# slyforce/MusicStyleTransfer

Measured on AMD Instinct MI355X. Metric: piano-roll frames/s (VAE train step), higher is better.
Workload: dtype bf16; 1 GPU; BASELINE configs[1]: single-track piano-roll VAE train step, T=256, pitch=128, latent=64, batch=64/GPU, bf16; encoder 256x2x8h, decoder 128x1x8h (scripts/train-vae.sh), dropout 0.2; Xavier-initialised weights; global_batch=64, seq_len=256, pitches=128, latent=64, parallelism=dp1, params=1885440

## Files before the change

include/mst_hip.h:

```cpp
#ifndef MST_HIP_H
#define MST_HIP_H

#include <stdint.h>

#ifdef __cplusplus
extern "C" {
#endif

typedef void* mst_stream_t;

enum mst_status {
  MST_OK = 0,
  MST_ERR_INVALID = -1,
  MST_ERR_LAUNCH = -2,
  MST_ERR_UNSUPPORTED = -3
};

enum mst_dtype { MST_BF16 = 0, MST_F16 = 1, MST_F32 = 2 };

enum mst_act { MST_ACT_NONE = 0, MST_ACT_RELU = 1 };

int mst_version(void);
const char* mst_last_error(void);
int mst_device_count(void);
// ... 135 lines not shown
                     int64_t S_out, int64_t s_off, const int32_t* idx, float* dst, int64_t ldd,
                     float alpha, mst_stream_t stream);

int mst_mask_from_lengths(int64_t B, int64_t S, const int32_t* lens, int32_t add,
                          uint8_t* keymask, mst_stream_t stream);

int mst_attn_keysoftmax_fwd(int dtype, int64_t B, int64_t S, int64_t H, int64_t dh,
                            const void* qkv, int64_t ld_qkv, int64_t k_off, int64_t q_off, int64_t v_off,
                            const uint8_t* keymask, float* lse,
                            void* out, int64_t ld_out,
                            int64_t q_limit ,
                            mst_stream_t stream);

int mst_attn_qkv_fwd(int dtype, int64_t B, int64_t S, int64_t H, int64_t dh, const void* x, int64_t ld_x, const void* w,
                     int64_t ld_w, const float* bias, void* qkv, int64_t ld_qkv, int64_t k_off, int64_t q_off, int64_t v_off,
                     const uint8_t* keymask, float* lse, void* out, int64_t ld_out, int64_t q_limit, mst_stream_t stream);
int mst_attn_keysoftmax_bwd(int dtype, int64_t B, int64_t S, int64_t H, int64_t dh,
                            const void* qkv, int64_t ld_qkv, int64_t k_off, int64_t q_off, int64_t v_off,
                            const uint8_t* keymask, const float* lse,
                            const void* dout, int64_t ld_dout,
                            void* dqkv, int64_t ld_dqkv, float* delta,
                            int64_t q_limit ,
                            mst_stream_t stream);

int mst_attn_causal_fwd(int dtype, int64_t B, int64_t S, int64_t H, int64_t dh,
                        const void* qkv, int64_t ld_qkv, int64_t k_off, int64_t q_off, int64_t v_off,
                        const uint8_t* keymask, float* lse, void* out, int64_t ld_out, mst_stream_t stream);
int mst_attn_causal_bwd(int dtype, int64_t B, int64_t S, int64_t H, int64_t dh,
                        const void* qkv, int64_t ld_qkv, int64_t k_off, int64_t q_off, int64_t v_off,
                        const uint8_t* keymask, const float* lse, const void* dout, int64_t ld_dout,
                        void* dqkv, int64_t ld_dqkv, float* delta, mst_stream_t stream);

int mst_layernorm_fwd(int dtype, int64_t M, int64_t D, const void* x, int64_t ldx,
                      const float* gamma, const float* beta, float eps,
                      void* y, int64_t ldy, float* mean, float* rstd,
                      int64_t row_id_stride ,
                      mst_stream_t stream);

int mst_layernorm_bwd(int dtype, int64_t M, int64_t D, const void* x, int64_t ldx,
                      const float* gamma, const float* mean, const float* rstd,
                      const void* dy, int64_t ldy, void* dx, int64_t ld_dx,
                      void* dx_masked, int64_t ld_dxm, float* dgamma, float* dbeta,
                      int mask_mode, float dropout_p, uint64_t dropout_seed, uint32_t dropout_site,
                      const uint64_t* dropout_seed_ptr,
                      int64_t row_id_stride ,
                      float* partials ,
// ... 191 lines not shown
```

musicstyletransfer_amd/_lib.py:

```python
import ctypes as C
import os

HERE = os.path.dirname(os.path.abspath(__file__))
LIB_PATH = os.path.join(HERE, "csrc", "libmst_hip.so")

MST_BF16, MST_F16, MST_F32 = 0, 1, 2
ACT_NONE, ACT_RELU = 0, 1
CE_MAX_WORKGROUPS = 4096

c_i32, c_i64, c_f32, c_f64, c_u64, c_u32 = C.c_int32, C.c_int64, C.c_float, C.c_double, C.c_uint64, C.c_uint32
vp = C.c_void_p


class GemmArgs(C.Structure):
    _fields_ = [
        ("dtype", c_i32), ("c_f32", c_i32),
        ("M", c_i64), ("N", c_i64), ("K", c_i64),
        ("A", vp), ("lda", c_i64),
        ("B", vp), ("ldb", c_i64),
        ("C", vp), ("ldc", c_i64),
        ("bias", vp),
        ("resid", vp), ("ldr", c_i64),
        ("act", c_i32),
        ("gate", vp), ("ldg", c_i64),
# ... 152 lines not shown
    "mst_gemm_wgrad": (C.c_int, [C.POINTER(WgradArgs), vp]),
    "mst_gemm_wgrad_batch": (C.c_int, [C.POINTER(WgradArgs), C.c_int, vp]),
    "mst_gemm_wgrad_batch_ws": (C.c_int, [C.POINTER(WgradArgs), C.c_int, vp, c_i64, vp]),
    "mst_gemm_wgrad_batch_sums": (C.c_int, [C.POINTER(WgradArgs), C.c_int, vp, c_i64, C.POINTER(PartialSum), C.c_int, vp]),
    "mst_gemm_wgrad_batch_flush": (C.c_int, [C.POINTER(WgradArgs), C.c_int, vp, c_i64, C.POINTER(PartialSum), C.c_int,
                                             C.POINTER(OuterJob), C.c_int, vp]),
    "mst_outer_jobs": (C.c_int, [C.POINTER(OuterJob), C.c_int, vp]),
    "mst_latent_bwd_vec": (C.c_int, [C.c_int, c_i64, c_i64, c_i64, c_i64, vp, vp, vp, vp, vp, vp, vp, c_i64, c_f32, c_f32, c_f32,
                                     c_f32, vp, c_i64, vp, c_i64, vp, vp]),
    "mst_latent_bwd_vec_proj": (C.c_int, [C.c_int, c_i64, c_i64, c_i64, c_i64, vp, vp, vp, vp, vp, vp, vp, c_i64, vp, c_i64, c_i64, vp, c_i64,
                                          c_f32, c_f32, c_f32, c_f32, vp, c_i64, vp, c_i64, vp, vp]),
    "mst_embed_fwd": (C.c_int, [C.c_int, c_i64, c_i64, c_i64, vp, vp, c_i64, vp, vp, c_i64, vp, c_i64, c_f32,
                                vp, c_i64, c_i64, c_i64, vp, vp]),
    "mst_embed_bwd": (C.c_int, [C.c_int, c_i64, c_i64, c_i64, vp, vp, c_i64, vp, vp, c_i64, c_f32,
                                vp, c_i64, c_i64, c_i64, vp]),
    "mst_group_colsum": (C.c_int, [C.c_int, c_i64, c_i64, c_i64, vp, c_i64, c_i64, c_i64, vp, vp, c_i64, c_f32, vp]),
    "mst_mask_from_lengths": (C.c_int, [c_i64, c_i64, vp, c_i32, vp, vp]),
    "mst_attn_keysoftmax_fwd": (C.c_int, [C.c_int, c_i64, c_i64, c_i64, c_i64, vp, c_i64, c_i64, c_i64, c_i64,
                                          vp, vp, vp, c_i64, c_i64, vp]),
    "mst_attn_qkv_fwd": (C.c_int, [C.c_int, c_i64, c_i64, c_i64, c_i64, vp, c_i64, vp, c_i64, vp, vp, c_i64, c_i64, c_i64, c_i64, vp, vp, vp,
                                   c_i64, c_i64, vp]),
    "mst_attn_keysoftmax_bwd": (C.c_int, [C.c_int, c_i64, c_i64, c_i64, c_i64, vp, c_i64, c_i64, c_i64, c_i64,
                                          vp, vp, vp, c_i64, vp, c_i64, vp, c_i64, vp]),
    "mst_attn_causal_fwd": (C.c_int, [C.c_int, c_i64, c_i64, c_i64, c_i64, vp, c_i64, c_i64, c_i64, c_i64, vp, vp, vp, c_i64, vp]),
    "mst_attn_causal_bwd": (C.c_int, [C.c_int, c_i64, c_i64, c_i64, c_i64, vp, c_i64, c_i64, c_i64, c_i64,
                                      vp, vp, vp, c_i64, vp, c_i64, vp, vp]),
    "mst_attn_decode": (C.c_int, [C.c_int, c_i64, c_i64, c_i64, c_i64, c_i64, vp, c_i64, c_i64, c_i64, c_i64, C.c_int, vp, c_i64, vp]),
    "mst_layernorm_fwd": (C.c_int, [C.c_int, c_i64, c_i64, vp, c_i64, vp, vp, c_f32, vp, c_i64, vp, vp, c_i64, vp]),
    "mst_layernorm_bwd": (C.c_int, [C.c_int, c_i64, c_i64, vp, c_i64, vp, vp, vp, vp, c_i64, vp, c_i64,
                                    vp, c_i64, vp, vp, C.c_int, c_f32, c_u64, c_u32, vp, c_i64, vp, vp]),
    "mst_latent_fwd": (C.c_int, [C.c_int, c_i64, c_i64, c_i64, c_i64, vp, c_i64, vp, vp, vp, vp, vp, vp, vp, c_i64,
                                 vp, c_f32, vp, vp, vp, vp, vp, c_i64, vp]),
    "mst_latent_fwd_proj": (C.c_int, [C.c_int, c_i64, c_i64, c_i64, c_i64, vp, c_i64, vp, vp, vp, vp, vp, vp, vp, c_i64,
                                      vp, c_f32, vp, vp, vp, vp, vp, c_i64, vp, c_i64, vp, vp, c_i64, c_i64, vp]),
    "mst_latent_bwd": (C.c_int, [C.c_int, c_i64, c_i64, c_i64, c_i64, vp, c_i64, vp, vp, vp, vp, vp, vp, vp,
                                 vp, c_i64, c_f32, c_f32, c_f32, c_f32, vp, vp, vp, vp, vp, c_i64, vp, c_i64, vp, vp]),
    "mst_reparam_kl_fwd": (C.c_int, [c_i64, c_i64, vp, vp, vp, vp, vp, vp]),
    "mst_reparam_kl_bwd": (C.c_int, [c_i64, c_i64, vp, vp, vp, vp, c_f32, vp, vp, vp]),
    "mst_softmax_ce": (C.c_int, [C.c_int, c_i64, c_i64, c_i64, vp, c_i64, vp, vp, vp, c_i64, vp, c_i64, c_f32, C.c_int, vp,
                                 C.c_int, vp]),
    "mst_ce_from_probs": (C.c_int, [C.c_int, c_i64, c_i64, c_i64, vp, c_i64, vp, vp, vp]),
    "mst_bce_from_probs": (C.c_int, [C.c_int, c_i64, c_i64, vp, vp, c_f32, C.c_int, vp, vp]),
    "mst_sigmoid_bce": (C.c_int, [C.c_int, c_i64, c_i64, c_i64, vp, c_i64, vp, c_f32, C.c_int, vp, vp, vp, c_i64,
                                  vp, c_i64, c_f32, C.c_int, vp]),
    "mst_beam_step": (C.c_int, [c_i64, c_i64, c_i64, c_i64, c_i64, vp, c_i64, vp, vp, vp, vp, vp, vp, vp, c_i32, c_i32, vp]),
    "mst_beam_gather": (C.c_int, [vp, vp, vp, c_i64, c_i64, c_i64, c_i64, vp]),
# ... 61 lines not shown
```

musicstyletransfer_amd/csrc/attention.hip:

```cpp
#include <math.h>
#include <stdlib.h>
#include <type_traits>
#include "common.hpp"

namespace mst {

#ifndef MST_ATT_STAGE
#define MST_ATT_STAGE 64
#endif
template <int DH> struct Stage { static constexpr int ROWS = MST_ATT_STAGE; };
template <int DH> struct LdsLd { static constexpr int V = DH + 8; };
constexpr int ATT_WG_ROWS = 128;
constexpr float MASK_VALUE = -1e9f;
constexpr float NEG_BIG = -3.0e38f;
constexpr float LOG2E = 1.4426950408889634f;

__device__ __forceinline__ void key_consts(bool in_range, bool valid_key, float rmax, float logl, float scale, float& sk2,
                                           float& ck2) {
  if (!in_range) { sk2 = 0.f; ck2 = -INFINITY; }
  else if (!valid_key) { sk2 = 0.f; ck2 = -logl * LOG2E; }
  else { sk2 = scale * LOG2E; ck2 = -(rmax + logl) * LOG2E; }
}
__device__ __forceinline__ float fast_exp2(float x) { return __builtin_amdgcn_exp2f(x); }
#define MST_FOR_TILES(kt, bits) for (uint64_t mst_m_ = (bits); mst_m_; mst_m_ &= mst_m_ - 1) if (const int kt = __builtin_ctzll(mst_m_); true)
// ... 832 lines not shown
    __syncthreads();
    LOOP_STAMP(6 + 5 * kc);
  }
  ATT_STAMP(1);
  if (!active) return;
  const bool in = row < S;
  T* const tiles[3] = {sK, sQ, sV};
  T* qrow = reinterpret_cast<T*>(const_cast<void*>(a.qkv)) + (b * S + row) * a.ld_qkv + hd * DH;
#pragma unroll
  for (int c = 0; c < 3; ++c) {
#pragma unroll
    for (int g = 0; g < 4; ++g) {
      u32x2 o = {0u, 0u};
      if (in) {
        o[0] = (uint32_t)f32_to_bits<T>(acc[c][4 * g]) | ((uint32_t)f32_to_bits<T>(acc[c][4 * g + 1]) << 16);
        o[1] = (uint32_t)f32_to_bits<T>(acc[c][4 * g + 2]) | ((uint32_t)f32_to_bits<T>(acc[c][4 * g + 3]) << 16);
        *reinterpret_cast<u32x2*>(qrow + sec_off[c] + 8 * g + h4) = o;
      }
      *reinterpret_cast<u32x2*>(tiles[c] + row * LD + 8 * g + h4) = o;
    }
  }
}

template <typename T, int DH, bool QKV = false, bool CHUNKED = false>
__global__ __launch_bounds__((FWD_MAX_WAVES<DH, QKV || CHUNKED> * 64)) __attribute__((amdgpu_waves_per_eu((DH == 16 ? MST_ATT16_WAVES_FWD : (FWD_MAX_WAVES<DH, QKV || CHUNKED> == 8 ? 2 : 4))))) void attn_fwd_res_kernel(AttnArgs a) {
  constexpr int KS = DH / 16, DB = (DH + 31) / 32, LD = LdsLd<DH>::V;
  extern __shared__ __attribute__((aligned(16))) unsigned char att_smem[];
  const int64_t S = a.S;
  const int NB = (int)((S + 31) / 32), SP = NB * 32;
  const bool restage = !QKV && a.restage;
  const int CR = CHUNKED ? SP / a.restage : SP;
  T* sQ = reinterpret_cast<T*>(att_smem);
  T* sK = restage ? sQ : sQ + SP * LD;
  T* sV = sK + CR * LD;
  float* sSk = reinterpret_cast<float*>(CHUNKED ? sQ + SP * LD : sV + SP * LD);
  float* sCk = sSk + SP; float* sMadd = sCk + SP; float* sMax = sMadd + SP; float* sLogl = sMax + SP;
  float* sRed = sLogl + SP;
  const int tid = threadIdx.x, lane = tid & 63, wave = tid >> 6, nthr = blockDim.x, NW = nthr >> 6;
  const int64_t bh = res_wg_bh(a.B, a.H), b = (int64_t)((uint32_t)bh / (uint32_t)a.H), hd = bh - b * a.H;
  const int64_t plane = a.B * a.H * S;
  const bool lone = lone_row_shape(S, DH) && a.q_limit >= S;
  const int NBo = lone ? NB - 1 : NB;
  const T* base = reinterpret_cast<const T*>(a.qkv) + b * S * a.ld_qkv + hd * DH;
  ATT_STAMP(0);
  if constexpr (QKV) {
    static_assert(DH == 32, "the fused projection is built for head size 32");
// ... 158 lines not shown
      for (int f = 0; f < DH; ++f) acc[f] = 0.f;
      for (int k = tid; k < S; k += nthr) {
        const float x = lds_row_dot<T, DH>(sK + k * LD, qe);
        const float p = exact ? exact_prob(x, a.scale, sMadd[k], sMax[k], sLogl[k]) : fast_exp2(fmaf(x, sSk[k], sCk[k]));
        lds_row_axpy<T, DH>(p, sV + k * LD, acc);
      }
#pragma unroll
      for (int f = 0; f < DH; ++f) acc[f] = wave_sum(acc[f]);
      if (lane == 0) {
#pragma unroll
        for (int f = 0; f < DH; ++f) sRed[wave * DH + f] = acc[f];
      }
      __syncthreads();
      if (tid < DH) {
        float o_e = 0.f;
        for (int w = 0; w < NW; ++w) o_e += sRed[w * DH + tid];
        T* og = reinterpret_cast<T*>(a.out) + b * S * a.ld_out + hd * DH;
        og[e * a.ld_out + tid] = (T)o_e;
      }
    }
  }
}

template <typename T, int DH, bool SPARSE>
__global__ __launch_bounds__(RES_MAX_WAVES<DH> * 64) __attribute__((amdgpu_waves_per_eu(DH == 16 ? MST_ATT16_WAVES_BWD : (DH == 64 ? 2 : 4)))) void attn_bwd_res_kernel(AttnArgs a) {
  constexpr int KS = DH / 16, DB = (DH + 31) / 32, LD = LdsLd<DH>::V;
  extern __shared__ __attribute__((aligned(16))) unsigned char att_smem[];
  const int64_t S = a.S;
  const int NB = (int)((S + 31) / 32), SP = NB * 32;
  T* bufA = reinterpret_cast<T*>(att_smem);
  T* bufB = bufA + SP * LD;
  float* sSk = reinterpret_cast<float*>(bufB + SP * LD);
  float* sCk = sSk + SP; float* sMadd = sCk + SP; float* sMax = sMadd + SP; float* sLogl = sMax + SP; float* sNd = sLogl + SP;
  float* sRed = sNd + SP;
  const int tid = threadIdx.x, lane = tid & 63, wave = tid >> 6, nthr = blockDim.x, NW = nthr >> 6;
  const int64_t bh = res_wg_bh(a.B, a.H), b = (int64_t)((uint32_t)bh / (uint32_t)a.H), hd = bh - b * a.H;
  const int64_t plane = a.B * a.H * S;
  const bool lone = !SPARSE && lone_row_shape(S, DH);
  const int NBo = lone ? NB - 1 : NB;
  const float log2_scale = __log2f(a.scale);
  const T* base = reinterpret_cast<const T*>(a.qkv) + b * S * a.ld_qkv + hd * DH;
  const T* Kg = base + a.k_off;
  const T* Qg = base + a.q_off;
  const T* Vg = base + a.v_off;
  const T* dOg = reinterpret_cast<const T*>(a.dout) + b * S * a.ld_dout + hd * DH;
  T* dbase = reinterpret_cast<T*>(a.dqkv) + b * S * a.ld_dqkv + hd * DH;
  constexpr bool sparse = SPARSE;
  const int64_t do_rows = sparse ? a.q_limit : S;
  typename Act<T>::vec8 kf[KS], vf[KS];
#pragma unroll
  for (int s = 0; s < KS; ++s) {
    kf[s] = glb_row_frag<T>(Kg, a.ld_qkv, wave * 32 + (lane & 31), S, s, lane);
    vf[s] = glb_row_frag<T>(Vg, a.ld_qkv, wave * 32 + (lane & 31), S, s, lane);
  }
  ATT_STAMP(0);
  stage_pair<T, DH>(bufA, Qg, a.ld_qkv, S, bufB, dOg, a.ld_dout, do_rows, SP, tid, nthr);
  __syncthreads();
  ATT_STAMP(1);
  const int nq0 = sparse ? 1 : NBo;

  int padded = 0;
  for (int ob = wave; ob < NBo; ob += NW) {
    const int64_t k_lane = ob * 32 + (lane & 31);
    if (ob != wave) {
#pragma unroll
      for (int s = 0; s < KS; ++s) {
        kf[s] = glb_row_frag<T>(Kg, a.ld_qkv, k_lane, S, s, lane);
        vf[s] = glb_row_frag<T>(Vg, a.ld_qkv, k_lane, S, s, lane);
      }
    }
    const bool in = k_lane < S;
    const bool vk = in && a.keymask[b * S + k_lane];
    const float rmax = in ? a.lse[bh * S + k_lane] : 0.f;
    const float logl = in ? a.lse[plane + bh * S + k_lane] : INFINITY;
    const float madd = vk ? 0.f : MASK_VALUE;
    float sk2, ck2;
    key_consts(in, vk, rmax, in ? logl : 0.f, a.scale, sk2, ck2);
    const float ck2s = ck2 + log2_scale;
    const bool exact_w = __any(in && !vk);
// ... 91 lines not shown
      }
      __syncthreads();
      if (tid < DH) {
        float dk = 0.f;
        for (int w = 0; w < NW; ++w) dk += sRed[w * DH + tid];
        dbase[e * a.ld_dqkv + a.k_off + tid] = (T)dk;
      }
      if (tid == 0) {
        a.delta[bh * S + e] = delta;
        sSk[e] = sk2; sCk[e] = ck2s; sMadd[e] = madd; sMax[e] = rmax; sLogl[e] = logl; sNd[e] = -delta;
        for (int k = (int)S; k < SP; ++k) {
          float s0, c0;
          key_consts(false, false, 0.f, 0.f, a.scale, s0, c0);
          sSk[k] = s0; sCk[k] = c0 + log2_scale; sMadd[k] = MASK_VALUE; sMax[k] = 0.f; sLogl[k] = INFINITY; sNd[k] = 0.f;
        }
      }
    }
  }
  ATT_STAMP(3);
  typename Act<T>::vec8 qf[KS], dof[KS];
#pragma unroll
  for (int s = 0; s < KS; ++s) {
    qf[s] = glb_row_frag<T>(Qg, a.ld_qkv, wave * 32 + (lane & 31), S, s, lane);
    dof[s] = glb_row_frag<T>(dOg, a.ld_dout, wave * 32 + (lane & 31), do_rows, s, lane);
  }
  __syncthreads();
  stage_pair<T, DH>(bufA, Kg, a.ld_qkv, S, bufB, Vg, a.ld_qkv, S, SP, tid, nthr);
  const bool exact = __syncthreads_or(padded);
  const uint64_t pad_tiles = exact ? padded_tile_mask(sSk, sCk, NB, lane) : 0ull;
  ATT_STAMP(4);

  for (int ob = wave; ob < NBo; ob += NW) {
    const int64_t q_lane = ob * 32 + (lane & 31);
    if (ob != wave) {
#pragma unroll
      for (int s = 0; s < KS; ++s) {
        qf[s] = glb_row_frag<T>(Qg, a.ld_qkv, q_lane, S, s, lane);
        dof[s] = glb_row_frag<T>(dOg, a.ld_dout, q_lane, do_rows, s, lane);
      }
    }
    f32x16 acc[DB];
#pragma unroll
    for (int d = 0; d < DB; ++d) acc[d] = zero16<DH>();
    if (sparse && ob > 0) {
      if (exact) {
        MST_FOR_TILES(kt, ~pad_tiles & tile_bits(NB)) bwd_q_tile<T, DH, false, true>(bufA, bufB, sSk, sCk, sMadd, sMax, sLogl, sNd, kt, a.scale, qf, dof, acc, lane);
        MST_FOR_TILES(kt, pad_tiles & tile_bits(NB)) bwd_q_tile<T, DH, true, true>(bufA, bufB, sSk, sCk, sMadd, sMax, sLogl, sNd, kt, a.scale, qf, dof, acc, lane);
      } else for (int kt = 0; kt < NB; ++kt) bwd_q_tile<T, DH, false, true>(bufA, bufB, sSk, sCk, sMadd, sMax, sLogl, sNd, kt, a.scale, qf, dof, acc, lane);
    } else if (exact) {
      MST_FOR_TILES(kt, ~pad_tiles & tile_bits(NBo)) bwd_q_tile<T, DH, false>(bufA, bufB, sSk, sCk, sMadd, sMax, sLogl, sNd, kt, a.scale, qf, dof, acc, lane);
      MST_FOR_TILES(kt, pad_tiles & tile_bits(NBo)) bwd_q_tile<T, DH, true>(bufA, bufB, sSk, sCk, sMadd, sMax, sLogl, sNd, kt, a.scale, qf, dof, acc, lane);
    } else {
      for (int kt = 0; kt < NBo; ++kt) bwd_q_tile<T, DH, false>(bufA, bufB, sSk, sCk, sMadd, sMax, sLogl, sNd, kt, a.scale, qf, dof, acc, lane);
    }
    if constexpr (DH <= 16 && !SPARSE) {
      if (lone) {
        if (exact) bwd_q_tile<T, DH, true, false, true>(bufA, bufB, sSk, sCk, sMadd, sMax, sLogl, sNd, NB - 1, a.scale, qf, dof, acc, lane);
        else bwd_q_tile<T, DH, false, false, true>(bufA, bufB, sSk, sCk, sMadd, sMax, sLogl, sNd, NB - 1, a.scale, qf, dof, acc, lane);
      }
    }
    owner_store<T, DH>(q_lane < S ? dbase + a.q_off + q_lane * a.ld_dqkv : nullptr, acc, lane);
  }
  ATT_STAMP(5);
  if constexpr (DH <= 16 && !SPARSE) {
    if (lone) {
      const int64_t e = S - 1;
      float qe[DH], doe[DH], acc[DH];
#pragma unroll
      for (int f = 0; f < DH; ++f) { qe[f] = to_f32(Qg[e * a.ld_qkv + f]); doe[f] = to_f32(dOg[e * a.ld_dout + f]); acc[f] = 0.f; }
      for (int k = tid; k < S; k += nthr) {
        const float x = lds_row_dot<T, DH>(bufA + k * LD, qe);
        const float ps = exact ? exact_prob(x, a.scale, sMadd[k], sMax[k], sLogl[k]) * a.scale : fast_exp2(fmaf(x, sSk[k], sCk[k]));
        const float dl = ps * (lds_row_dot<T, DH>(bufB + k * LD, doe) + sNd[k]);
        lds_row_axpy<T, DH>(dl, bufA + k * LD, acc);
      }
#pragma unroll
      for (int f = 0; f < DH; ++f) acc[f] = wave_sum(acc[f]);
      if (lane == 0) {
#pragma unroll
        for (int f = 0; f < DH; ++f) sRed[wave * DH + f] = acc[f];
      }
      __syncthreads();
      if (tid < DH) {
        float dq = 0.f;
        for (int w = 0; w < NW; ++w) dq += sRed[w * DH + tid];
        dbase[e * a.ld_dqkv + a.q_off + tid] = (T)dq;
      }
    }
  }
}

template <typename T, int DH, int OBM>
// ... 212 lines not shown
    const int NB = (int)cdiv(a.S, 32);
    if (!off && DH == 32 && NB <= OBM * NWQ) {
      for (int nc = 1; nc <= 4; nc *= 2) {
        if (NB % nc != 0) break;
        const size_t lds = (size_t)2 * (NB * 32 / nc) * LdsLd<DH>::V * 2 + (size_t)6 * NB * 32 * 4;
        if (lds > 150 * 1024) continue;
        static size_t attr_lds = 64 * 1024;
        if (lds > attr_lds) {
          const hipError_t e = hipFuncSetAttribute(reinterpret_cast<const void*>(&attn_bwd_q_chunk_kernel<T, DH, OBM>), hipFuncAttributeMaxDynamicSharedMemorySize, (int)lds);
          if (e != hipSuccess) { set_error("attn_bwd_q_chunk_kernel: LDS opt-in of %zu bytes: %s", lds, hipGetErrorString(e)); return MST_ERR_LAUNCH; }
          attr_lds = lds;
        }
        hipLaunchKernelGGL((attn_bwd_q_chunk_kernel<T, DH, OBM>), dim3((unsigned)(a.B * a.H)), dim3(NWQ * 64), lds, s, a, nc);
        MST_CHECK_LAUNCH("attn_bwd_q_chunk_kernel");
        return MST_OK;
      }
    }
  }
  hipLaunchKernelGGL((attn_bwd_q_kernel<T, DH>), grid, dim3(256), 0, s, a);
  MST_CHECK_LAUNCH("attn_bwd_q_kernel");
  return MST_OK;
}


template <typename T, int DH>
__global__ __launch_bounds__(64) void attn_decode_kernel(int64_t H, int64_t n_keys, int64_t t_max, const T* __restrict__ cache,
                                                          int64_t ld, int64_t k_off, int64_t q_off, int64_t v_off, int mode,
                                                          float scale, T* __restrict__ out, int64_t ld_out) {
  const int64_t b = blockIdx.x / H, hd = blockIdx.x % H;
  const int lane = threadIdx.x;
  const T* base = cache + b * t_max * ld + hd * DH;
  float q[DH];
#pragma unroll
  for (int d = 0; d < DH; ++d) q[d] = to_f32(base[(n_keys - 1) * ld + q_off + d]);
  float m = -INFINITY;
  if (mode == 1) {
    for (int64_t k = lane; k < n_keys; k += 64) {
      float l = 0.f;
#pragma unroll
      for (int d = 0; d < DH; ++d) l = fmaf(to_f32(base[k * ld + k_off + d]), q[d], l);
      m = fmaxf(m, l * scale);
    }
    m = wave_max(m);
  }
  float acc[DH], z = 0.f;
#pragma unroll
// ... 88 lines not shown
extern "C" int mst_attn_keysoftmax_bwd(int dtype, int64_t B, int64_t S, int64_t H, int64_t dh, const void* qkv,
                                       int64_t ld_qkv, int64_t k_off, int64_t q_off, int64_t v_off,
                                       const uint8_t* keymask, const float* lse, const void* dout, int64_t ld_dout,
                                       void* dqkv, int64_t ld_dqkv, float* delta, int64_t q_limit, mst_stream_t stream) {
  int rc = attn_check(B, S, H, dh, ld_qkv, k_off, q_off, v_off);
  if (rc) return rc;
  MST_CHECK_ARG(qkv && keymask && lse && dout && dqkv && delta, "mst_attn_keysoftmax_bwd: null pointer");
  MST_CHECK_ARG(ld_dout % 8 == 0 && ld_dout >= H * dh && ld_dqkv % 8 == 0, "mst_attn_keysoftmax_bwd: bad leading dims");
  AttnArgs a = {};
  a.B = B; a.S = S; a.H = H; a.qkv = qkv; a.ld_qkv = ld_qkv; a.k_off = k_off; a.q_off = q_off; a.v_off = v_off;
  a.keymask = keymask; a.lse = const_cast<float*>(lse); a.dout = dout; a.ld_dout = ld_dout; a.dqkv = dqkv;
  a.ld_dqkv = ld_dqkv; a.delta = delta;
  a.q_limit = (q_limit > 0 && q_limit < S) ? q_limit : 0;
  a.scale = 1.f / sqrtf((float)dh);
  hipStream_t s = (hipStream_t)stream;
  return dispatch_act(dtype, [&](auto tag) -> int {
    typedef decltype(tag) T;
    if (dh == 16) return launch_bwd<T, 16>(a, s);
    if (dh == 32) return launch_bwd<T, 32>(a, s);
    return launch_bwd<T, 64>(a, s);
  });
}

extern "C" int mst_attn_decode(int dtype, int64_t B, int64_t H, int64_t dh, int64_t n_keys, int64_t t_max, const void* cache,
                               int64_t ld, int64_t k_off, int64_t q_off, int64_t v_off, int mode, void* out, int64_t ld_out,
                               mst_stream_t stream) {
  MST_CHECK_ARG(B > 0 && H > 0 && n_keys > 0 && n_keys <= t_max && cache && out, "mst_attn_decode: bad argument");
  MST_CHECK_ARG(dh == 16 || dh == 32 || dh == 64, "mst_attn_decode: head size must be 16, 32 or 64 (got %lld)", (long long)dh);
  MST_CHECK_ARG(mode == 0 || mode == 1, "mst_attn_decode: mode must be 0 (softmax over the query axis, the reference) or 1 (over the keys)");
  MST_CHECK_ARG(ld_out >= H * dh, "mst_attn_decode: ld_out < H*dh");
  const float scale = 1.f / sqrtf((float)dh);
  hipStream_t s = (hipStream_t)stream;
  return dispatch_act(dtype, [&](auto tag) -> int {
    typedef decltype(tag) T;
    const dim3 grid((unsigned)(B * H));
    if (dh == 16) hipLaunchKernelGGL((attn_decode_kernel<T, 16>), grid, dim3(64), 0, s, H, n_keys, t_max, (const T*)cache, ld, k_off, q_off, v_off, mode, scale, (T*)out, ld_out);
    else if (dh == 32) hipLaunchKernelGGL((attn_decode_kernel<T, 32>), grid, dim3(64), 0, s, H, n_keys, t_max, (const T*)cache, ld, k_off, q_off, v_off, mode, scale, (T*)out, ld_out);
    else hipLaunchKernelGGL((attn_decode_kernel<T, 64>), grid, dim3(64), 0, s, H, n_keys, t_max, (const T*)cache, ld, k_off, q_off, v_off, mode, scale, (T*)out, ld_out);
    MST_CHECK_LAUNCH("attn_decode_kernel");
    return MST_OK;
  });
}
```

musicstyletransfer_amd/engine.py:

```python
import math
import os
import warnings
from collections import OrderedDict

import numpy as np
import torch

from . import ops as o


def roundup(a, b):
    return (a + b - 1) // b * b


def _lib_ce_rows():
    from . import _lib
    return _lib.CE_MAX_WORKGROUPS


class VAEConfig:

    def __init__(self, kind, in_dim, out_dim, num_classes, latent_dim, e_model, e_layers, e_heads, d_model, d_layers,
                 d_heads, e_dropout=0.0, d_dropout=0.0, d_causal=False):
        assert kind in ("token", "pianoroll")
# ... 873 lines not shown
                                st.grad(f"{pre}.ln3.beta"), D=D, mask_mode=2, dropout_site=site0 + 2,
                                partials=self._ln_partials(f"{pre}.ln3", o.layernorm_bwd_parts(M, D)), **dk)
            dff = t.dh
            resid_ff = None
        ln1 = dict(dx_masked=t.dh1m, mask_mode=1, dropout_site=site0, **dk) if p > 0 else {}
        if ffn_fused:
            rows = self._row0_groups(side, i)
            o.ffn_ln_bwd(dff, st.t(f"{pre}.ff2.weight"), t.dpre, L.a, st.t(f"{pre}.ff1.weight"), t.dh1, L.h1, st.p(f"{pre}.ln1.gamma"),
                         L.mean1, L.rstd1, st.grad(f"{pre}.ln1.gamma"), st.grad(f"{pre}.ln1.beta"), alpha=inv_keep, resid=resid_ff,
                         partials=self._ln_partials(f"{pre}.ln1", o.gemm_nt_ln_parts(self.B * self.T if rows else M)), lead=lead,
                         row_groups=rows, **ln1)
        else:
            o.gemm_nt(dff, st.t(f"{pre}.ff2.weight"), t.dpre, N=4 * D, K=D, gate=L.a, alpha=inv_keep)
            if fuse:
                o.gemm_nt_ln_bwd(t.dpre, st.t(f"{pre}.ff1.weight"), t.dh1, L.h1, st.p(f"{pre}.ln1.gamma"), L.mean1, L.rstd1,
                                 st.grad(f"{pre}.ln1.gamma"), st.grad(f"{pre}.ln1.beta"), N=D, K=4 * D, resid=resid_ff,
                                 partials=self._ln_partials(f"{pre}.ln1", o.gemm_nt_ln_parts(M)), **ln1)
            else:
                o.gemm_nt(t.dpre, st.t(f"{pre}.ff1.weight"), t.dx1, N=D, K=4 * D, resid=resid_ff)
                o.layernorm_bwd(L.h1, st.p(f"{pre}.ln1.gamma"), L.mean1, L.rstd1, t.dx1, t.dh1, st.grad(f"{pre}.ln1.gamma"),
                                st.grad(f"{pre}.ln1.beta"), D=D, partials=self._ln_partials(f"{pre}.ln1", o.layernorm_bwd_parts(M, D)),
                                **ln1)
        dproj = t.dh1m if p > 0 else t.dh1
        o.gemm_nt(dproj, st.t(f"{pre}.att.W_proj.weight"), t.datt, N=D, K=D)
        if side == "decoder" and self.cfg.d_causal:
            o.attn_causal_bwd(L.qkv, keymask, L.lse, t.datt, t.dqkv, t.delta, self.B, S, H, dhd, 0, D, 2 * D)
        else:
            o.attn_bwd(L.qkv, keymask, L.lse, t.datt, t.dqkv, t.delta, self.B, S, H, dhd, 0, D, 2 * D)
        if next_ln is not None:
            kw, t_below = next_ln
            o.gemm_nt_ln_bwd(t.dqkv, st.t(f"{pre}.att.W_kqv"), t_below.dh, N=D, K=3 * D, resid=t.dh1, **kw)
        elif side == "decoder" and i == 0 and self._ride_bwd_planned():
            T_ = self.T
            self._bwd_rider = dict(A=t.dqkv, B=st.t(f"{pre}.att.W_kqv"), C_out=dx_in, M=self.B * T_, N=D, K=3 * D, resid=t.dh1, resid_phys=True,
                                   a_remap=(T_, T_ + 1, 1), c_remap=(T_, T_ + 1, 1))
            self._bwd_dx0 = (t.dqkv.view(self.B, S, -1), st.t(f"{pre}.att.W_kqv"), t.dh1.view(self.B, S, -1))
        else:
            o.gemm_nt(t.dqkv, st.t(f"{pre}.att.W_kqv"), dx_in, N=D, K=3 * D, resid=t.dh1)
        self._wgrads += [
            o.wgrad_problem(dff, L.a, st.grad(f"{pre}.ff2.weight"), st.grad(f"{pre}.ff2.bias"), N=D, K=4 * D),
            o.wgrad_problem(t.dpre, L.x1, st.grad(f"{pre}.ff1.weight"), st.grad(f"{pre}.ff1.bias"), N=4 * D, K=D),
            o.wgrad_problem(dproj, L.att, st.grad(f"{pre}.att.W_proj.weight"), st.grad(f"{pre}.att.W_proj.bias"), N=D, K=D),
            o.wgrad_problem(t.dqkv, x_in, st.fused(st.g, pre, "weight"), st.fused(st.g, pre, "bias"), N=3 * D, K=D),
        ]

    def _top_encoder_layer_bwd(self, i, L, x_in, dx_in, t, next_ln=None):
        cfg, st, B, S = self.cfg, self.store, self.B, self.T
        D, H, p, site0 = cfg.e_model, cfg.e_heads, cfg.e_dropout, self._site_e(i)
        pre = f"encoder.layer{i}"
        c = self.top
        inv_keep = 1.0 / (1.0 - p) if p > 0 else 1.0
# ... 244 lines not shown
```

musicstyletransfer_amd/ops.py:

```python
import ctypes as C
import math

import torch

from . import _lib
from ._lib import LnArgs, LnBwdIn, PartialSum, OuterJob, StepBeginArgs, StepMetrics, ACT_NONE, ACT_RELU, MST_BF16, MST_F16, GemmArgs, WgradArgs, call

_DT = {torch.bfloat16: MST_BF16, torch.float16: MST_F16}


def dt(x):
    try:
        return _DT[x if isinstance(x, torch.dtype) else x.dtype]
    except KeyError:
        raise TypeError(f"activation dtype must be bfloat16 or float16, got {x}") from None


def ptr(t):
    if t is None:
        return None
    assert t.is_cuda, "mst ops need device tensors (there is no CPU fallback)"
    if t.device.index != torch.cuda.current_device():
        raise RuntimeError(f"tensor on cuda:{t.device.index} but the current device is cuda:{torch.cuda.current_device()}: "
                           "call torch.cuda.set_device() for this rank's GPU first")
# ... 338 lines not shown
    if outers:
        outer_jobs(outers)


def gemm_wgrad(A, B, dW, db=None, **kw):
    gemm_wgrad_batch([wgrad_problem(A, B, dW, db, **kw)])


def attn_fwd(qkv, keymask, lse, out, B, S, H, dh, k_off, q_off, v_off, q_limit=0):
    call("mst_attn_keysoftmax_fwd", dt(qkv), B, S, H, dh, ptr(qkv), ld(qkv), k_off, q_off, v_off, ptr(keymask),
         ptr(lse), ptr(out), ld(out), q_limit, stream())


def attn_qkv_fwd(x, W, bias, qkv, keymask, lse, out, B, S, H, dh, k_off, q_off, v_off, q_limit=0):
    call("mst_attn_qkv_fwd", dt(qkv), B, S, H, dh, ptr(x), ld(x), ptr(W), ld(W), ptr(bias), ptr(qkv), ld(qkv), k_off, q_off, v_off,
         ptr(keymask), ptr(lse), ptr(out), ld(out), q_limit, stream())


def attn_bwd(qkv, keymask, lse, dout, dqkv, delta, B, S, H, dh, k_off, q_off, v_off, q_limit=0):
    call("mst_attn_keysoftmax_bwd", dt(qkv), B, S, H, dh, ptr(qkv), ld(qkv), k_off, q_off, v_off, ptr(keymask),
         ptr(lse), ptr(dout), ld(dout), ptr(dqkv), ld(dqkv), ptr(delta), q_limit, stream())


def attn_causal_fwd(qkv, keymask, lse, out, B, S, H, dh, k_off, q_off, v_off):
    call("mst_attn_causal_fwd", dt(qkv), B, S, H, dh, ptr(qkv), ld(qkv), k_off, q_off, v_off, ptr(keymask), ptr(lse), ptr(out),
         ld(out), stream())


def attn_causal_bwd(qkv, keymask, lse, dout, dqkv, delta, B, S, H, dh, k_off, q_off, v_off):
    call("mst_attn_causal_bwd", dt(qkv), B, S, H, dh, ptr(qkv), ld(qkv), k_off, q_off, v_off, ptr(keymask), ptr(lse), ptr(dout),
         ld(dout), ptr(dqkv), ld(dqkv), ptr(delta), stream())


def attn_decode(cache3, n_keys, H, dh, k_off, q_off, v_off, out, mode=0):
    B, t_max = cache3.shape[0], cache3.shape[1]
    assert cache3.stride(2) == 1 and cache3.stride(0) == t_max * cache3.stride(1)
    call("mst_attn_decode", dt(cache3), B, H, dh, n_keys, t_max, ptr(cache3), cache3.stride(1), k_off, q_off, v_off, mode, ptr(out),
         ld(out), stream())


def beam_step(probs, scores_in, scores_out, seqs_in, seqs_out, hyp_src, word, i, K, eos, pad, active=None):
    N, V = probs.shape[0], probs.shape[1]
    call("mst_beam_step", N // K, K, V, i, seqs_in.shape[1], ptr(probs), probs.stride(0), ptr(scores_in), ptr(scores_out), ptr(seqs_in),
         ptr(seqs_out), ptr(hyp_src), ptr(word), ptr(active), eos, pad, stream())


# ... 292 lines not shown
```

Baseline: 25.82 million frames/s.

## Fuse attention output-projection backward GEMM into the dense attention backward kernel

Adds a prologue to the resident attention backward kernel that computes each head's slice of dproj·W_proj in LDS with MFMA. The dO operand then comes from LDS instead of a separate GEMM writing datt to global memory. This removes one GEMM launch and the datt round trip for the non-causal layers with head size 16 or 32, and falls back to GEMM plus the old kernel otherwise. The cost is that each block recomputes its projection slice over the full model width, which adds LDS pressure and per-block serial work before the attention math.

```diff
diff --git a/include/mst_hip.h b/include/mst_hip.h
--- a/include/mst_hip.h
+++ b/include/mst_hip.h
@@ -181,6 +181,10 @@
                             void* dqkv, int64_t ld_dqkv, float* delta,
                             int64_t q_limit ,
                             mst_stream_t stream);
+int mst_attn_proj_bwd(int dtype, int64_t B, int64_t S, int64_t H, int64_t dh, const void* dproj, int64_t ld_dproj,
+                      const void* wpt, int64_t ld_wpt, const void* qkv, int64_t ld_qkv, int64_t k_off, int64_t q_off,
+                      int64_t v_off, const uint8_t* keymask, const float* lse, void* dout, int64_t ld_dout, void* dqkv,
+                      int64_t ld_dqkv, float* delta, int64_t q_limit, mst_stream_t stream);
 
 int mst_attn_causal_fwd(int dtype, int64_t B, int64_t S, int64_t H, int64_t dh,
                         const void* qkv, int64_t ld_qkv, int64_t k_off, int64_t q_off, int64_t v_off,
diff --git a/musicstyletransfer_amd/_lib.py b/musicstyletransfer_amd/_lib.py
--- a/musicstyletransfer_amd/_lib.py
+++ b/musicstyletransfer_amd/_lib.py
@@ -198,6 +198,8 @@
                                    c_i64, c_i64, vp]),
     "mst_attn_keysoftmax_bwd": (C.c_int, [C.c_int, c_i64, c_i64, c_i64, c_i64, vp, c_i64, c_i64, c_i64, c_i64,
                                           vp, vp, vp, c_i64, vp, c_i64, vp, c_i64, vp]),
+    "mst_attn_proj_bwd": (C.c_int, [C.c_int, c_i64, c_i64, c_i64, c_i64, vp, c_i64, vp, c_i64, vp, c_i64, c_i64, c_i64, c_i64,
+                                    vp, vp, vp, c_i64, vp, c_i64, vp, c_i64, vp]),
     "mst_attn_causal_fwd": (C.c_int, [C.c_int, c_i64, c_i64, c_i64, c_i64, vp, c_i64, c_i64, c_i64, c_i64, vp, vp, vp, c_i64, vp]),
     "mst_attn_causal_bwd": (C.c_int, [C.c_int, c_i64, c_i64, c_i64, c_i64, vp, c_i64, c_i64, c_i64, c_i64,
                                       vp, vp, vp, c_i64, vp, c_i64, vp, vp]),
diff --git a/musicstyletransfer_amd/csrc/attention.hip b/musicstyletransfer_amd/csrc/attention.hip
--- a/musicstyletransfer_amd/csrc/attention.hip
+++ b/musicstyletransfer_amd/csrc/attention.hip
@@ -878,6 +878,90 @@
   }
 }
 
+template <int DH> constexpr int PROJ_KC = DH == 32 ? 64 : 32;
+template <int DH> constexpr int PROJ_XP = DH == 32 ? 4 : 3;
+template <int DH>
+__host__ __device__ inline size_t proj_lds_bytes(int64_t SP) { return ((size_t)SP + DH) * (PROJ_KC<DH> + 8) * 2; }
+template <typename T, int DH>
+__device__ __forceinline__ void proj_bwd_prologue(const AttnArgs& a, T* lds, T* sdO, int64_t b, int64_t hd, int NB) {
+  constexpr int KC = PROJ_KC<DH>, XL = KC + 8, CPR = KC / 8, XP = PROJ_XP<DH>, LD = LdsLd<DH>::V;
+  const int tid = threadIdx.x, lane = tid & 63, wave = tid >> 6, nthr = blockDim.x, NW = nthr >> 6;
+  const int64_t S = a.S;
+  const int SP = NB * 32;
+  T* const sX = lds;
+  T* const sW = lds + SP * XL;
+  const T* xg = reinterpret_cast<const T*>(a.x) + b * S * a.ld_x;
+  const T* wg = reinterpret_cast<const T*>(a.w) + hd * DH * a.ld_w;
+  const int nch = (int)(a.Dm / KC);
+  const T* xsrc[XP]; T* xdst[XP]; bool xok[XP];
+#pragma unroll
+  for (int i = 0; i < XP; ++i) {
+    const int p = tid + i * nthr;
+    xok[i] = p < SP * CPR;
+    const int r = xok[i] ? p / CPR : 0, ch = xok[i] ? p % CPR : 0;
+    xsrc[i] = xg + (int64_t)(r < S ? r : S - 1) * a.ld_x + ch * 8;
+    xdst[i] = sX + r * XL + ch * 8;
+  }
+  const bool wok = tid < DH * CPR;
+  const int wr_ = wok ? tid / CPR : 0, wch = wok ? tid % CPR : 0;
+  const T* const wsrc = wg + (int64_t)wr_ * a.ld_w + wch * 8;
+  T* const wdst = sW + wr_ * XL + wch * 8;
+  u32x4 xr[XP], wrg;
+  auto load_slice = [&](int kc) {
+    const int k = (kc < nch ? kc : nch - 1) * KC;
+#pragma unroll
+    for (int i = 0; i < XP; ++i) xr[i] = *reinterpret_cast<const u32x4*>(xsrc[i] + k);
+    wrg = *reinterpret_cast<const u32x4*>(wsrc + k);
+  };
+  auto store_slice = [&]() {
+#pragma unroll
+    for (int i = 0; i < XP; ++i)
+      if (xok[i]) *reinterpret_cast<u32x4*>(xdst[i]) = xr[i];
+    if (wok) *reinterpret_cast<u32x4*>(wdst) = wrg;
+  };
+  const int ob1 = wave + NW;
+  const bool two = ob1 < NB;
+  f32x16 acc0 = zero16<DH>(), acc1 = zero16<DH>();
+  load_slice(0);
+  store_slice();
+  __syncthreads();
+  const bool wlane = (lane & 31) < DH;
+  const T* const fw = sW + (wlane ? (lane & 31) : 0) * XL + 8 * (lane >> 5);
+  const T* const fx0 = sX + (wave * 32 + (lane & 31)) * XL + 8 * (lane >> 5);
+  const T* const fx1 = sX + ((two ? ob1 : wave) * 32 + (lane & 31)) * XL + 8 * (lane >> 5);
+  for (int kc = 0; kc < nch; ++kc) {
+    load_slice(kc + 1);
+#pragma unroll
+    for (int s4 = 0; s4 < KC / 16; ++s4) {
+      u32x4 wv = *reinterpret_cast<const u32x4*>(fw + 16 * s4);
+      if (!wlane) wv = u32x4{0u, 0u, 0u, 0u};
+      const typename Act<T>::vec8 wf = __builtin_bit_cast(typename Act<T>::vec8, wv);
+      acc0 = Act<T>::mfma32(wf, __builtin_bit_cast(typename Act<T>::vec8, *reinterpret_cast<const u32x4*>(fx0 + 16 * s4)), acc0);
+      if (two) acc1 = Act<T>::mfma32(wf, __builtin_bit_cast(typename Act<T>::vec8, *reinterpret_cast<const u32x4*>(fx1 + 16 * s4)), acc1);
+    }
+    __syncthreads();
+    if (kc + 1 < nch) store_slice();
+    __syncthreads();
+  }
+  const int h4 = 4 * (lane >> 5);
+  auto put = [&](const f32x16& acc, int ob) {
+    const int64_t row = (int64_t)ob * 32 + (lane & 31);
+    const bool in = row < S;
+#pragma unroll
+    for (int g = 0; g < 4; ++g)
+      if (8 * g < DH) {
+        u32x2 o = {0u, 0u};
+        if (in) {
+          o[0] = (uint32_t)f32_to_bits<T>(acc[4 * g]) | ((uint32_t)f32_to_bits<T>(acc[4 * g + 1]) << 16);
+          o[1] = (uint32_t)f32_to_bits<T>(acc[4 * g + 2]) | ((uint32_t)f32_to_bits<T>(acc[4 * g + 3]) << 16);
+        }
+        *reinterpret_cast<u32x2*>(sdO + row * LD + 8 * g + h4) = o;
+      }
+  };
+  if (wave < NB) put(acc0, wave);
+  if (two) put(acc1, ob1);
+}
+
 template <typename T, int DH, bool QKV = false, bool CHUNKED = false>
 __global__ __launch_bounds__((FWD_MAX_WAVES<DH, QKV || CHUNKED> * 64)) __attribute__((amdgpu_waves_per_eu((DH == 16 ? MST_ATT16_WAVES_FWD : (FWD_MAX_WAVES<DH, QKV || CHUNKED> == 8 ? 2 : 4))))) void attn_fwd_res_kernel(AttnArgs a) {
   constexpr int KS = DH / 16, DB = (DH + 31) / 32, LD = LdsLd<DH>::V;
@@ -1082,8 +1166,9 @@
   }
 }
 
-template <typename T, int DH, bool SPARSE>
+template <typename T, int DH, bool SPARSE, bool PROJ = false>
 __global__ __launch_bounds__(RES_MAX_WAVES<DH> * 64) __attribute__((amdgpu_waves_per_eu(DH == 16 ? MST_ATT16_WAVES_BWD : (DH == 64 ? 2 : 4)))) void attn_bwd_res_kernel(AttnArgs a) {
+  static_assert(!PROJ || (!SPARSE && DH <= 32), "the fused projection is for the dense kernel at head sizes 16 and 32");
   constexpr int KS = DH / 16, DB = (DH + 31) / 32, LD = LdsLd<DH>::V;
   extern __shared__ __attribute__((aligned(16))) unsigned char att_smem[];
   const int64_t S = a.S;
@@ -1103,18 +1188,23 @@
   const T* Kg = base + a.k_off;
   const T* Qg = base + a.q_off;
   const T* Vg = base + a.v_off;
-  const T* dOg = reinterpret_cast<const T*>(a.dout) + b * S * a.ld_dout + hd * DH;
+  const T* dOg = PROJ ? nullptr : reinterpret_cast<const T*>(a.dout) + b * S * a.ld_dout + hd * DH;
   T* dbase = reinterpret_cast<T*>(a.dqkv) + b * S * a.ld_dqkv + hd * DH;
   constexpr bool sparse = SPARSE;
   const int64_t do_rows = sparse ? a.q_limit : S;
   typename Act<T>::vec8 kf[KS], vf[KS];
+  if constexpr (PROJ) proj_bwd_prologue<T, DH>(a, bufA, bufB, b, hd, NB);
 #pragma unroll
   for (int s = 0; s < KS; ++s) {
     kf[s] = glb_row_frag<T>(Kg, a.ld_qkv, wave * 32 + (lane & 31), S, s, lane);
     vf[s] = glb_row_frag<T>(Vg, a.ld_qkv, wave * 32 + (lane & 31), S, s, lane);
   }
   ATT_STAMP(0);
-  stage_pair<T, DH>(bufA, Qg, a.ld_qkv, S, bufB, dOg, a.ld_dout, do_rows, SP, tid, nthr);
+  if constexpr (PROJ) {
+    stage_all<T, DH>(bufA, Qg, a.ld_qkv, S, SP, tid, nthr);
+  } else {
+    stage_pair<T, DH>(bufA, Qg, a.ld_qkv, S, bufB, dOg, a.ld_dout, do_rows, SP, tid, nthr);
+  }
   __syncthreads();
   ATT_STAMP(1);
   const int nq0 = sparse ? 1 : NBo;
@@ -1252,7 +1342,12 @@
 #pragma unroll
   for (int s = 0; s < KS; ++s) {
     qf[s] = glb_row_frag<T>(Qg, a.ld_qkv, wave * 32 + (lane & 31), S, s, lane);
-    dof[s] = glb_row_frag<T>(dOg, a.ld_dout, wave * 32 + (lane & 31), do_rows, s, lane);
+    if constexpr (PROJ) dof[s] = wave < NB ? lds_row_frag<T, DH>(bufB, wave * 32, s, lane) : typename Act<T>::vec8{};
+    else dof[s] = glb_row_frag<T>(dOg, a.ld_dout, wave * 32 + (lane & 31), do_rows, s, lane);
+  }
+  float* const sLoneDo = sRed + LONE_RED / 2 + 32;
+  if constexpr (PROJ && DH <= 16) {
+    if (lone && tid < DH) sLoneDo[tid] = to_f32(bufB[(S - 1) * LD + tid]);
   }
   __syncthreads();
   stage_pair<T, DH>(bufA, Kg, a.ld_qkv, S, bufB, Vg, a.ld_qkv, S, SP, tid, nthr);
@@ -1262,7 +1357,7 @@
 
   for (int ob = wave; ob < NBo; ob += NW) {
     const int64_t q_lane = ob * 32 + (lane & 31);
-    if (ob != wave) {
+    if (!PROJ && ob != wave) {
 #pragma unroll
       for (int s = 0; s < KS; ++s) {
         qf[s] = glb_row_frag<T>(Qg, a.ld_qkv, q_lane, S, s, lane);
@@ -1297,7 +1392,7 @@
       const int64_t e = S - 1;
       float qe[DH], doe[DH], acc[DH];
 #pragma unroll
-      for (int f = 0; f < DH; ++f) { qe[f] = to_f32(Qg[e * a.ld_qkv + f]); doe[f] = to_f32(dOg[e * a.ld_dout + f]); acc[f] = 0.f; }
+      for (int f = 0; f < DH; ++f) { qe[f] = to_f32(Qg[e * a.ld_qkv + f]); doe[f] = PROJ ? sLoneDo[f] : to_f32(dOg[e * a.ld_dout + f]); acc[f] = 0.f; }
       for (int k = tid; k < S; k += nthr) {
         const float x = lds_row_dot<T, DH>(bufA + k * LD, qe);
         const float ps = exact ? exact_prob(x, a.scale, sMadd[k], sMax[k], sLogl[k]) * a.scale : fast_exp2(fmaf(x, sSk[k], sCk[k]));
@@ -1556,6 +1651,29 @@
   return MST_OK;
 }
 
+template <typename T, int DH>
+static int launch_bwd_proj(const AttnArgs& a, hipStream_t s) {
+  const char* off = getenv("MST_ATTN_PROJ_BWD");
+  if ((off && off[0] == '0') || a.q_limit != 0) return 0;
+  const size_t lds = res_lds_bwd<DH>(a.S);
+  const bool lone = lone_row_shape(a.S, DH);
+  const int nw = choose_resident(a.S, a.B * a.H, lds, DH == 16 ? 4 * MST_ATT16_WAVES_BWD : RES_MAX_WAVES<DH>, lone, RES_MAX_WAVES<DH>);
+  const int NB = (int)cdiv(a.S, 32), NBo = NB - (lone ? 1 : 0);
+  constexpr int KC = PROJ_KC<DH>, CPR = KC / 8;
+  if (!nw || nw < NBo || NB > 2 * nw || a.Dm % KC != 0 || NB * 32 * CPR > PROJ_XP<DH> * nw * 64 || DH * CPR > nw * 64 ||
+      proj_lds_bytes<DH>(NB * 32) > lds)
+    return 0;
+  static size_t attr_lds = 64 * 1024;
+  if (lds > attr_lds) {
+    const hipError_t e = hipFuncSetAttribute(reinterpret_cast<const void*>(&attn_bwd_res_kernel<T, DH, false, true>),
+                                             hipFuncAttributeMaxDynamicSharedMemorySize, (int)lds);
+    if (e != hipSuccess) { set_error("attn_bwd_res_kernel (fused projection): LDS opt-in of %zu bytes: %s", lds, hipGetErrorString(e)); return MST_ERR_LAUNCH; }
+    attr_lds = lds;
+  }
+  hipLaunchKernelGGL((attn_bwd_res_kernel<T, DH, false, true>), dim3((unsigned)(a.B * a.H)), dim3(nw * 64), lds, s, a);
+  MST_CHECK_LAUNCH("attn_bwd_res_kernel (fused projection)");
+  return 1;
+}
 
 template <typename T, int DH>
 __global__ __launch_bounds__(64) void attn_decode_kernel(int64_t H, int64_t n_keys, int64_t t_max, const T* __restrict__ cache,
@@ -1690,6 +1808,42 @@
   });
 }
 
+extern "C" int mst_attn_proj_bwd(int dtype, int64_t B, int64_t S, int64_t H, int64_t dh, const void* dproj, int64_t ld_dproj,
+                                 const void* wpt, int64_t ld_wpt, const void* qkv, int64_t ld_qkv, int64_t k_off, int64_t q_off,
+                                 int64_t v_off, const uint8_t* keymask, const float* lse, void* dout, int64_t ld_dout, void* dqkv,
+                                 int64_t ld_dqkv, float* delta, int64_t q_limit, mst_stream_t stream) {
+  int rc = attn_check(B, S, H, dh, ld_qkv, k_off, q_off, v_off);
+  if (rc) return rc;
+  const int64_t Dm = H * dh;
+  MST_CHECK_ARG(dproj && wpt && qkv && keymask && lse && dout && dqkv && delta, "mst_attn_proj_bwd: null pointer");
+  MST_CHECK_ARG(ld_dproj % 8 == 0 && ld_dproj >= Dm && ld_wpt % 8 == 0 && ld_wpt >= Dm && ld_dout % 8 == 0 && ld_dout >= Dm &&
+                ld_dqkv % 8 == 0, "mst_attn_proj_bwd: leading dimensions must be multiples of 8 and cover the model width");
+  MST_CHECK_ARG(((uintptr_t)dproj % 16 == 0) && ((uintptr_t)wpt % 16 == 0) && ((uintptr_t)qkv % 16 == 0) && ((uintptr_t)dqkv % 16 == 0),
+                "mst_attn_proj_bwd: operands must be 16-byte aligned");
+  hipStream_t s = (hipStream_t)stream;
+  if (dh <= 32) {
+    AttnArgs a = {};
+    a.B = B; a.S = S; a.H = H; a.qkv = qkv; a.ld_qkv = ld_qkv; a.k_off = k_off; a.q_off = q_off; a.v_off = v_off;
+    a.keymask = keymask; a.lse = const_cast<float*>(lse); a.dout = nullptr; a.ld_dout = 0; a.dqkv = dqkv;
+    a.ld_dqkv = ld_dqkv; a.delta = delta;
+    a.q_limit = (q_limit > 0 && q_limit < S) ? q_limit : 0;
+    a.scale = 1.f / sqrtf((float)dh);
+    a.x = dproj; a.ld_x = ld_dproj; a.w = wpt; a.ld_w = ld_wpt; a.Dm = Dm;
+    rc = dispatch_act(dtype, [&](auto tag) -> int {
+      typedef decltype(tag) T;
+      return dh == 16 ? launch_bwd_proj<T, 16>(a, s) : launch_bwd_proj<T, 32>(a, s);
+    });
+    if (rc != 0) return rc < 0 ? rc : MST_OK;
+  }
+  mst_gemm_args g = {};
+  g.dtype = dtype; g.M = B * S; g.N = Dm; g.K = Dm;
+  g.A = dproj; g.lda = ld_dproj; g.B = wpt; g.ldb = ld_wpt; g.C = dout; g.ldc = ld_dout; g.alpha = 1.f;
+  rc = mst_gemm_nt(&g, stream);
+  if (rc) return rc;
+  return mst_attn_keysoftmax_bwd(dtype, B, S, H, dh, qkv, ld_qkv, k_off, q_off, v_off, keymask, lse, dout, ld_dout, dqkv, ld_dqkv,
+                                 delta, q_limit, stream);
+}
+
 extern "C" int mst_attn_decode(int dtype, int64_t B, int64_t H, int64_t dh, int64_t n_keys, int64_t t_max, const void* cache,
                                int64_t ld, int64_t k_off, int64_t q_off, int64_t v_off, int mode, void* out, int64_t ld_out,
                                mst_stream_t stream) {
diff --git a/musicstyletransfer_amd/engine.py b/musicstyletransfer_amd/engine.py
--- a/musicstyletransfer_amd/engine.py
+++ b/musicstyletransfer_amd/engine.py
@@ -919,11 +919,12 @@
                                 st.grad(f"{pre}.ln1.beta"), D=D, partials=self._ln_partials(f"{pre}.ln1", o.layernorm_bwd_parts(M, D)),
                                 **ln1)
         dproj = t.dh1m if p > 0 else t.dh1
-        o.gemm_nt(dproj, st.t(f"{pre}.att.W_proj.weight"), t.datt, N=D, K=D)
         if side == "decoder" and self.cfg.d_causal:
+            o.gemm_nt(dproj, st.t(f"{pre}.att.W_proj.weight"), t.datt, N=D, K=D)
             o.attn_causal_bwd(L.qkv, keymask, L.lse, t.datt, t.dqkv, t.delta, self.B, S, H, dhd, 0, D, 2 * D)
         else:
-            o.attn_bwd(L.qkv, keymask, L.lse, t.datt, t.dqkv, t.delta, self.B, S, H, dhd, 0, D, 2 * D)
+            o.attn_proj_bwd(dproj, st.t(f"{pre}.att.W_proj.weight"), L.qkv, keymask, L.lse, t.datt, t.dqkv, t.delta, self.B, S, H, dhd,
+                            0, D, 2 * D)
         if next_ln is not None:
             kw, t_below = next_ln
             o.gemm_nt_ln_bwd(t.dqkv, st.t(f"{pre}.att.W_kqv"), t_below.dh, N=D, K=3 * D, resid=t.dh1, **kw)
diff --git a/musicstyletransfer_amd/ops.py b/musicstyletransfer_amd/ops.py
--- a/musicstyletransfer_amd/ops.py
+++ b/musicstyletransfer_amd/ops.py
@@ -384,6 +384,11 @@
          ptr(lse), ptr(dout), ld(dout), ptr(dqkv), ld(dqkv), ptr(delta), q_limit, stream())
 
 
+def attn_proj_bwd(dproj, Wpt, qkv, keymask, lse, dout, dqkv, delta, B, S, H, dh, k_off, q_off, v_off, q_limit=0):
+    call("mst_attn_proj_bwd", dt(qkv), B, S, H, dh, ptr(dproj), ld(dproj), ptr(Wpt), ld(Wpt), ptr(qkv), ld(qkv), k_off, q_off, v_off,
+         ptr(keymask), ptr(lse), ptr(dout), ld(dout), ptr(dqkv), ld(dqkv), ptr(delta), q_limit, stream())
+
+
 def attn_causal_fwd(qkv, keymask, lse, out, B, S, H, dh, k_off, q_off, v_off):
     call("mst_attn_causal_fwd", dt(qkv), B, S, H, dh, ptr(qkv), ld(qkv), k_off, q_off, v_off, ptr(keymask), ptr(lse), ptr(out),
          ld(out), stream())
```

Measured after the change: 26.11 million frames/s (median of 6 runs). +1.1%, better.
